# FraVirgu/Parallel-Geometric-Multigrid-for-Poisson-problem

Hardware: NVIDIA B200
Metric: V-cycle GDOF/s to 1e-8 residual (higher is better)
Workload: dtype f64

## Files before the change

### parallel-geometric-multigrid-for-poisson-problem_b200/csrc/kernels_fused.cu

```cuda
#include <cstdlib>
#include <cstring>

#define PMG_NEEDS_PEER_WAIT
#include "pmg_internal.h"

namespace pmg {

namespace {

constexpr int WARPS_PER_CTA = 4;

__host__ __device__ constexpr int halo_for(int stages) { return stages <= 4 ? 4 : 8; }

struct StripGeom {
    int n;
    int ny;
    int yoff;
    int row_lo;
    int row_hi;
    int pitch;
    int n_strips;
    int n_chunks;
    int chunk_rows;
    int halo;
// ... 125 lines not shown
        cen[p ^ 1] = in;
        return out;
    }
    template <bool WEIGHTED>
    __device__ __forceinline__ Row<C> step_wide(const int p, const Row<C> &in, const Row<C> &h2f, const JacobiCoef &c,
                                                bool keep0, bool keep_row)
    {
        static_assert(C == 4, "wide geometry: 4 columns per lane");
        Row<C> out, w, e;
        const Row<C> &prev = cen[p];
#pragma unroll
        for (int k = 0; k < C; ++k) {
            const double sum = dadd(part.v[k], in.v[k]);
            double val = WEIGHTED ? dadd(dmul(c.om1, prev.v[k]), dmul(c.w4, sum)) : dmul(0.25, sum);
            out.v[k] = ((k == 0) ? keep0 : keep_row) ? prev.v[k] : val;
        }
        neighbours<C>(in, w, e);
#pragma unroll
        for (int k = 0; k < C; ++k) part.v[k] = dadd(dadd(dadd(h2f.v[k], w.v[k]), e.v[k]), prev.v[k]);
        cen[p ^ 1] = in;
        return out;
    }
};

template <int C>
struct ResidualStage {
    Row<C> part;
    Row<C> cen[2];
    __device__ __forceinline__ void init()
    {
        cen[0] = zero_row<C>();
        cen[1] = zero_row<C>();
        part = zero_row<C>();
    }
    __device__ __forceinline__ Row<C> step(const int p, const Row<C> &in, const Row<C> &f_prev, double inv_h2)
    {
        Row<C> r, w, e;
#pragma unroll
        for (int k = 0; k < C; ++k)
            r.v[k] = dsub(f_prev.v[k], dmul(inv_h2, dsub(part.v[k], in.v[k])));
        neighbours<C>(in, w, e);
#pragma unroll
        for (int k = 0; k < C; ++k)
            part.v[k] = dsub(dsub(dfma_pow2(4.0, in.v[k], -w.v[k]), e.v[k]), cen[p].v[k]);
        cen[p ^ 1] = in;
        return r;
// ... 266 lines not shown
struct FeedSelect<C, PF, S, USE_X, true> {
    using type = SmemFeed<C, PF, S, USE_X>;
};

template <int C>
struct CoarseRow {
    double v[C / 2 + 1];
};

template <int C>
__device__ __forceinline__ CoarseRow<C> load_coarse(const double *__restrict__ p)
{
    CoarseRow<C> r;
    if (C == 4) {
        const double2 t = __ldg(reinterpret_cast<const double2 *>(p));
        r.v[0] = t.x;
        r.v[1] = t.y;
    } else {
        r.v[0] = __ldg(p);
    }
    return r;
}

template <int C, int PF, int MINB, bool SM, int S, bool ZEROX, bool RESID, bool WEIGHTED, bool PROLOGUE = false, bool PIN = false>
__global__ void __launch_bounds__(32 * WARPS_PER_CTA, MINB)
    k_down(const double *__restrict__ x, double *__restrict__ xo, const double *__restrict__ f,
           double *__restrict__ cf, StripGeom g, int pitch_c, int nc, JacobiCoef coef, double inv_h2,
           const int *__restrict__ done, HaloPeers hp, const double *__restrict__ e_in, int pitch_e, int lo)
{
    static_assert(!PIN || (ZEROX && SM), "prolong-in: the iterate is not read, shared-memory feed (row pairs)");
    using Feed = typename FeedSelect<C, PF, S, !ZEROX, SM>::type;
    pdl_wait();
    const bool pdl_early = gridDim.x <= 296u;
    if (pdl_early) pdl_trigger();
    if (done != nullptr && *done) return;
    constexpr int NP = C / 2;
    const int wid = __shfl_sync(0xffffffffu, (int)((blockIdx.x * (unsigned)blockDim.x + threadIdx.x) >> 5), 0);
    const int lane = threadIdx.x & 31;
    if (wid >= g.n_strips * g.n_chunks) return;
    int col, r0, r1;
    bool owner, cin[C];
    strip_setup<C>(g, wid, lane, col, r0, r1, owner, cin);

    const int lead = RESID ? 2 : 0;
    int j_start_ = min(r0, max(r0, 0) - lead) - S;
    if (PIN) j_start_ -= (j_start_ & 1);
    const int j_start = j_start_;
    const int j_end = max(r1 - 1, min(r1, g.ny) - 1 + (RESID ? 1 : 0)) + S;

    SweepStage<C> st[S];
    ResidualStage<C> rs;
#pragma unroll
    for (int k = 0; k < S; ++k) st[k].init();
    rs.init();
    double s_mid[NP], s_cor[NP], c_mid[NP], c_ew[NP];
#pragma unroll
    for (int q = 0; q < NP; ++q) s_mid[q] = s_cor[q] = c_mid[q] = c_ew[q] = 0.0;

    const int epoch = hp.epoch + (hp.epoch_base != nullptr ? *hp.epoch_base : 0);
    if ((hp.pub_up != nullptr || hp.pub_dn != nullptr) && blockIdx.x == 0 && threadIdx.x == 0) {
        __threadfence_system();
        if (hp.pub_up != nullptr) publish_epoch(hp.pub_up, epoch);
        if (hp.pub_dn != nullptr) publish_epoch(hp.pub_dn, epoch);
    }
    HaloPeers feed_peers = hp;
    if constexpr (!PROLOGUE) {
        if (hp.flag_up != nullptr || hp.flag_dn != nullptr) {
            int ok = 1;
            if (lane == 0) {
                if (hp.flag_up != nullptr) ok = wait_flag(hp.flag_up, epoch) ? ok : 0;
                if (hp.flag_dn != nullptr) ok = wait_flag(hp.flag_dn, epoch) ? ok : 0;
// ... 68 lines not shown
                double corr[C];
                if ((u & 1) == 0) {
                    en = eb;
                    en.v[NP] = __shfl_down_sync(0xffffffffu, eb.v[0], 1);
                    const int nr = min((jj >> 1) + 2, nc_last_row);
                    eb = load_coarse<C>(e_in + (ptrdiff_t)nr * pitch_e + cc);
#pragma unroll
                    for (int q = 0; q < NP; ++q) {
                        corr[2 * q] = ec.v[q];
                        corr[2 * q + 1] = dadd(ec.v[q], ec.v[q + 1]);
                    }
                } else {
#pragma unroll
                    for (int q = 0; q < NP; ++q) {
                        corr[2 * q] = dadd(ec.v[q], en.v[q]);
                        corr[2 * q + 1] = dadd(dadd(dadd(ec.v[q], ec.v[q + 1]), en.v[q]), en.v[q + 1]);
                    }
                    ec = en;
                }
#pragma unroll
                for (int k = 0; k < C; ++k)
                    if (rowp && cprol[k]) cur.v[k] = add_correction(cur.v[k], corr[k], u & 1, k & 1);
            }
#pragma unroll
            for (int k = 0; k < S; ++k) {
                const int out_row = jj - k - 1 + g.yoff;
                cur = st[k].template step<WEIGHTED>(u & 1, cur, feed.f_row(k), coef, out_row > 0 && out_row < g.n - 1, cin);
            }
            const int xrow = jj - S;
            if (owner && xrow >= r0 && xrow < r1) store_row<C>(xo + (ptrdiff_t)xrow * g.pitch + col, cur);
            if (RESID) {
                Row<C> r = rs.step(u & 1, cur, feed.f_row(S + 1), inv_h2);
                const int rrow = jj - S - 1;
                double left = __shfl_up_sync(0xffffffffu, r.v[C - 1], 1);
                if (rrow & 1) {
                    const int jc = (rrow - 1) >> 1;
                    const int ic = col >> 1;
                    double o[NP];
#pragma unroll
                    for (int q = 0; q < NP; ++q) {
                        double west = (q == 0) ? left : r.v[q == 0 ? 0 : 2 * q - 1];
                        double edge = dadd(dadd(c_ew[q], r.v[2 * q]), s_mid[q]);
                        double corner = dadd(dadd(s_cor[q], west), r.v[2 * q + 1]);
                        double val = dfma_pow2(0.0625, corner, dfma_pow2(0.125, edge, dmul(0.25, c_mid[q])));
                        o[q] = (ic + q >= 1 && ic + q < nc - 1) ? val : 0.0;
                        s_mid[q] = r.v[2 * q];
                        s_cor[q] = dadd(west, r.v[2 * q + 1]);
                    }
                    if (owner && jc + ycoarse >= 1 && jc + ycoarse < nc - 1 && 2 * jc >= r0 && 2 * jc < r1 &&
                        jc >= 0 && 2 * jc < g.ny) {
                        double *dst = cf + (ptrdiff_t)jc * pitch_c + ic;
                        if (NP == 2)
                            *reinterpret_cast<double2 *>(dst) = make_double2(o[0], o[NP - 1]);
                        else
                            *dst = o[0];
                    }
                } else {
#pragma unroll
                    for (int q = 0; q < NP; ++q) {
                        double west = (q == 0) ? left : r.v[q == 0 ? 0 : 2 * q - 1];
                        c_mid[q] = r.v[2 * q];
                        c_ew[q] = dadd(r.v[2 * q + 1], west);
                    }
                }
            }
            feed.end();
        }
    }
    if (!pdl_early) pdl_trigger();
    cp_async_wait<0>();
}

template <int C, int PF, int MINB, bool SM, int S, bool PROLONG, bool NORM, bool WEIGHTED>
__global__ void __launch_bounds__(32 * WARPS_PER_CTA, MINB)
    k_up(const double *__restrict__ xb, double *__restrict__ xo, const double *__restrict__ f,
         const double *__restrict__ e, StripGeom g, int pitch_c, int lo, JacobiCoef coef, double inv_h2,
         double *__restrict__ partials, const int *__restrict__ done)
{
    using Feed = typename FeedSelect<C, PF, S, true, SM>::type;
    pdl_wait();
    const bool pdl_early = gridDim.x <= 296u;
    if (pdl_early) pdl_trigger();
    if (done != nullptr && *done) return;
    static_assert(Feed::UNROLL % 2 == 0, "rows are processed in (even, odd) pairs");
    constexpr int NP = C / 2;
    const int wid = __shfl_sync(0xffffffffu, (int)((blockIdx.x * (unsigned)blockDim.x + threadIdx.x) >> 5), 0);
    const int lane = threadIdx.x & 31;
    if (wid >= g.n_strips * g.n_chunks) return;
    int col, r0, r1;
    bool owner, cin[C];
    strip_setup<C>(g, wid, lane, col, r0, r1, owner, cin);

    int j_start = r0 - S - (NORM ? 1 : 0);
    j_start -= (j_start & 1);
    const int j_end = r1 - 1 + S + (NORM ? 1 : 0);

    SweepStage<C> st[S];
    ResidualStage<C> rs;
#pragma unroll
    for (int k = 0; k < S; ++k) st[k].init();
    rs.init();
    double acc = 0.0;

    bool cprol[C];
#pragma unroll
    for (int k = 0; k < C; ++k) cprol[k] = (col + k >= lo) && (col + k <= g.n - 2);

    Feed feed;
    feed.init(xb, f, g.pitch, col, j_start, g.ny + PADY - 1, lane, threadIdx.x >> 5, HaloPeers{}, g.ny);

    const int cc = col >> 1;
    const int nc_last_row = ((g.ny - 1) >> 1) + PADY;
    CoarseRow<C> ec, en, eb;
#pragma unroll
    for (int q = 0; q <= NP; ++q) ec.v[q] = en.v[q] = eb.v[q] = 0.0;
    if (PROLONG) {
        const int jc0 = j_start >> 1;
        ec = load_coarse<C>(e + (ptrdiff_t)jc0 * pitch_c + cc);
        ec.v[NP] = __shfl_down_sync(0xffffffffu, ec.v[0], 1);
        eb = load_coarse<C>(e + (ptrdiff_t)(jc0 + 1) * pitch_c + cc);
    }

    for (int j = j_start; j <= j_end; j += Feed::UNROLL) {
#pragma unroll
        for (int u = 0; u < Feed::UNROLL; ++u) {
            const int jj = j + u;
            Row<C> cur = feed.begin(u, jj);
            if (PROLONG) {
                const bool rowp = (jj + g.yoff >= lo) && (jj + g.yoff <= g.n - 2);
                double corr[C];
                if ((u & 1) == 0) {
                    en = eb;
                    en.v[NP] = __shfl_down_sync(0xffffffffu, eb.v[0], 1);
                    int nr = min((jj >> 1) + 2, nc_last_row);
                    eb = load_coarse<C>(e + (ptrdiff_t)nr * pitch_c + cc);
#pragma unroll
                    for (int q = 0; q < NP; ++q) {
                        corr[2 * q] = ec.v[q];
                        corr[2 * q + 1] = dadd(ec.v[q], ec.v[q + 1]);
                    }
                } else {
#pragma unroll
                    for (int q = 0; q < NP; ++q) {
                        corr[2 * q] = dadd(ec.v[q], en.v[q]);
                        corr[2 * q + 1] = dadd(dadd(dadd(ec.v[q], ec.v[q + 1]), en.v[q]), en.v[q + 1]);
                    }
                    ec = en;
                }
#pragma unroll
                for (int k = 0; k < C; ++k)
                    if (rowp && cprol[k]) cur.v[k] = add_correction(cur.v[k], corr[k], u & 1, k & 1);
            }
#pragma unroll
            for (int k = 0; k < S; ++k) {
                const int out_row = jj - k - 1 + g.yoff;
                cur = st[k].template step<WEIGHTED>(u & 1, cur, feed.f_row(k), coef, out_row > 0 && out_row < g.n - 1, cin);
            }
            const int xrow = jj - S;
            if (owner && xrow >= r0 && xrow < r1) store_row<C>(xo + (ptrdiff_t)xrow * g.pitch + col, cur);
            if (NORM) {
                Row<C> r = rs.step(u & 1, cur, feed.f_row(S + 1), inv_h2);
                const int rrow = jj - S - 1;
                if (owner && rrow >= r0 && rrow < r1 && rrow >= 0 && rrow < g.ny && rrow + g.yoff > 0 &&
                    rrow + g.yoff < g.n - 1) {
#pragma unroll
                    for (int k = 0; k < C; ++k)
                        if (cin[k]) acc = dadd(acc, dmul(r.v[k], r.v[k]));
                }
            }
            feed.end();
        }
    }
    if (!pdl_early) pdl_trigger();
    cp_async_wait<0>();
    if (NORM) {
#pragma unroll
        for (int o = 16; o > 0; o >>= 1) acc = dadd(acc, __shfl_xor_sync(0xffffffffu, acc, o));
        if (lane == 0) partials[wid] = acc;
    }
}

template <int C, int PF, int MINB, int S2, int S1, bool WEIGHTED, bool GEN_F = false>
__global__ void __launch_bounds__(32 * WARPS_PER_CTA, MINB)
    k_cross(const double *__restrict__ xb, double *__restrict__ xo, double *__restrict__ xk, const double *__restrict__ f,
// ... 289 lines not shown
#endif

inline int current_device()
{
#ifdef PMG_HOST_EMULATION
    return 0;
#else
    int d = 0;
    cudaGetDevice(&d);
    return d & 63;
#endif
}
#define PMG_SMEM_ONCE(k, sm)                         \
    do {                                             \
        static unsigned long long mask_ = 0;         \
        const int d_ = current_device();             \
        if (!((mask_ >> d_) & 1ull)) {               \
            set_smem(k, sm);                         \
            mask_ |= 1ull << d_;                     \
        }                                            \
    } while (0)

template <int C, int PF, int MINB, bool SM, int S, bool WEIGHTED>
void down_launch_w(const FusedLevel &lv, double *cf, int pitch_c, bool x_is_zero, bool resid, const StripGeom &g,
                   int nc, const JacobiCoef &c, double inv, dim3 grid, dim3 block, const int *done, cudaStream_t st)
{
    constexpr bool CAN_PROLOGUE = SM && S == 2;
    const bool prologue = CAN_PROLOGUE && g_halo_prologue && (lv.hp.flag_up != nullptr || lv.hp.flag_dn != nullptr);
    if (resid && x_is_zero && prologue) {
        auto k = k_down<C, PF, MINB, SM, S, true, true, WEIGHTED, CAN_PROLOGUE>;
        int sm = WARPS_PER_CTA * FeedSelect<C, PF, S, false, SM>::type::SMEM_PER_WARP;
        PMG_SMEM_ONCE(k, sm);
        PMG_LAUNCH(k, grid, block, sm, st, lv.x, lv.xb, lv.f, cf, g, pitch_c, nc, c, inv, done, lv.hp, (const double *)nullptr, 0, 0);
    } else if (resid && prologue) {
        auto k = k_down<C, PF, MINB, SM, S, false, true, WEIGHTED, CAN_PROLOGUE>;
        int sm = WARPS_PER_CTA * FeedSelect<C, PF, S, true, SM>::type::SMEM_PER_WARP;
        PMG_SMEM_ONCE(k, sm);
        PMG_LAUNCH(k, grid, block, sm, st, lv.x, lv.xb, lv.f, cf, g, pitch_c, nc, c, inv, done, lv.hp, (const double *)nullptr, 0, 0);
    } else if (resid && x_is_zero) {
        auto k = k_down<C, PF, MINB, SM, S, true, true, WEIGHTED>;
        int sm = WARPS_PER_CTA * FeedSelect<C, PF, S, false, SM>::type::SMEM_PER_WARP;
        PMG_SMEM_ONCE(k, sm);
        PMG_LAUNCH(k, grid, block, sm, st, lv.x, lv.xb, lv.f, cf, g, pitch_c, nc, c, inv, done, lv.hp, (const double *)nullptr, 0, 0);
    } else if (resid) {
        auto k = k_down<C, PF, MINB, SM, S, false, true, WEIGHTED>;
        int sm = WARPS_PER_CTA * FeedSelect<C, PF, S, true, SM>::type::SMEM_PER_WARP;
        PMG_SMEM_ONCE(k, sm);
        PMG_LAUNCH(k, grid, block, sm, st, lv.x, lv.xb, lv.f, cf, g, pitch_c, nc, c, inv, done, lv.hp, (const double *)nullptr, 0, 0);
    } else {
        auto k = k_down<C, PF, MINB, SM, S, false, false, WEIGHTED>;
        int sm = WARPS_PER_CTA * FeedSelect<C, PF, S, true, SM>::type::SMEM_PER_WARP;
        PMG_SMEM_ONCE(k, sm);
        PMG_LAUNCH(k, grid, block, sm, st, lv.x, lv.xb, lv.f, (double *)nullptr, g, 0, nc, c, inv, done, lv.hp, (const double *)nullptr, 0, 0);
    }
}

template <int C, int PF, int MINB, bool SM, int S>
void down_launch(const FusedLevel &lv, double *cf, int pitch_c, double omega, bool x_is_zero, bool resid,
                 const int *done, cudaStream_t st)
{
    StripGeom g = make_geom(lv, S + (resid ? 2 : 0), VariantDesc{C, PF, MINB, SM}, lv.ext_lo, lv.ext_hi);
    JacobiCoef c = jacobi_coef(lv.h, omega);
    double inv = 1.0 / (lv.h * lv.h);
    int nc = (lv.n - 1) / 2 + 1;
    dim3 grid(grid_for(g)), block(32 * WARPS_PER_CTA);
    if (c.weighted) {
        down_launch_w<C, PF, MINB, SM, S, true>(lv, cf, pitch_c, x_is_zero, resid, g, nc, c, inv, grid, block, done, st);
    } else {
        down_launch_w<C, PF, MINB, SM, S, false>(lv, cf, pitch_c, x_is_zero, resid, g, nc, c, inv, grid, block, done, st);
    }
    count_launch();
}

template <bool WEIGHTED>
void down_prolong_launch_w(const FusedLevel &lv, const double *e_in, int pitch_e, int lo, double *cf, int pitch_c,
                           const JacobiCoef &c, const int *done, cudaStream_t st)
{
    constexpr int C = 2, PF = 3, MINB = 5, S = 2;
    StripGeom g = make_geom(lv, S + 2, VariantDesc{C, PF, MINB, 1}, lv.ext_lo, lv.ext_hi);
    const double inv = 1.0 / (lv.h * lv.h);
    const int nc = (lv.n - 1) / 2 + 1;
    auto k = k_down<C, PF, MINB, true, S, true, true, WEIGHTED, false, true>;
    int sm = WARPS_PER_CTA * SmemFeed<C, PF, S, false>::SMEM_PER_WARP;
    PMG_SMEM_ONCE(k, sm);
    PMG_LAUNCH(k, dim3(grid_for(g)), dim3(32 * WARPS_PER_CTA), sm, st, lv.x, lv.xb, lv.f, cf, g, pitch_c, nc, c, inv, done,
               HaloPeers{}, e_in, pitch_e, lo);
}

template <int C, int PF, int MINB, bool SM, int S, bool PROLONG, bool NORM, bool WEIGHTED>
void up_launch_k(const FusedLevel &lv, const double *e, int pitch_c, const StripGeom &g, int lo,
                 const JacobiCoef &c, double inv, double *d_partials, const int *done, cudaStream_t st)
{
    auto k = k_up<C, PF, MINB, SM, S, PROLONG, NORM, WEIGHTED>;
    int sm = WARPS_PER_CTA * FeedSelect<C, PF, S, true, SM>::type::SMEM_PER_WARP;
    PMG_SMEM_ONCE(k, sm);
    PMG_LAUNCH(k, dim3(grid_for(g)), dim3(32 * WARPS_PER_CTA), sm, st, lv.xb, lv.x, lv.f, e, g, pitch_c, lo, c, inv, d_partials, done);
}

template <int C, int PF, int MINB, bool SM, int S, bool PROLONG, bool NORM>
void up_launch_one(const FusedLevel &lv, const double *e, int pitch_c, const StripGeom &g, int lo,
                   const JacobiCoef &c, double inv, double *d_partials, const int *done, cudaStream_t st)
{
    if (c.weighted)
        up_launch_k<C, PF, MINB, SM, S, PROLONG, NORM, true>(lv, e, pitch_c, g, lo, c, inv, d_partials, done, st);
    else
        up_launch_k<C, PF, MINB, SM, S, PROLONG, NORM, false>(lv, e, pitch_c, g, lo, c, inv, d_partials, done, st);
}

template <int C, int PF, int MINB, bool SM, int S>
void up_launch(const FusedLevel &lv, const double *e, int pitch_c, double omega, int lo, bool norm,
               double *d_partials, int *n_partials, const int *done, cudaStream_t st)
{
    StripGeom g = make_geom(lv, S + (norm ? 2 : 1), VariantDesc{C, PF, MINB, SM}, lv.ext_lo, lv.ext_hi);
    JacobiCoef c = jacobi_coef(lv.h, omega);
    double inv = 1.0 / (lv.h * lv.h);
    if (e != nullptr) {
        if (norm)
            up_launch_one<C, PF, MINB, SM, S, true, true>(lv, e, pitch_c, g, lo, c, inv, d_partials, done, st);
        else
            up_launch_one<C, PF, MINB, SM, S, true, false>(lv, e, pitch_c, g, lo, c, inv, d_partials, done, st);
    } else {
        if (norm)
            up_launch_one<C, PF, MINB, SM, S, false, true>(lv, e, pitch_c, g, lo, c, inv, d_partials, done, st);
        else
            up_launch_one<C, PF, MINB, SM, S, false, false>(lv, e, pitch_c, g, lo, c, inv, d_partials, done, st);
    }
    count_launch();
    if (n_partials) *n_partials = norm ? g.n_strips * g.n_chunks : 0;
}

template <int C, int PF, int MINB, bool WEIGHTED, bool GEN_F = false>
void cross_launch_w(const FusedLevel &lv_in, double *xb_out, const double *e, int pitch_c, double *cf, int lo, double *d_partials,
                    int *n_partials, const JacobiCoef &c, const int *done, cudaStream_t st)
{
    VariantDesc v{C, PF, MINB, 1};
    StripGeom g = make_geom(lv_in, 6, v, 0, 0, C == 2 ? 6 : 8);
    double inv = 1.0 / (lv_in.h * lv_in.h);
    int nc = (lv_in.n - 1) / 2 + 1;
    auto k = k_cross<C, PF, MINB, 2, 2, WEIGHTED, GEN_F>;
    int sm = WARPS_PER_CTA * SmemFeed<C, PF, 4, true, GEN_F, C == 4>::SMEM_PER_WARP;
    PMG_SMEM_ONCE(k, sm);
    PMG_LAUNCH(k, dim3(grid_for(g)), dim3(32 * WARPS_PER_CTA), sm, st, lv_in.xb, xb_out, lv_in.x, lv_in.f, e, cf, g, pitch_c, lo, nc, c,
               inv, d_partials, done, lv_in.hp, lv_in.rhs_fx, lv_in.rhs_sy);
    if (n_partials) *n_partials = g.n_strips * g.n_chunks;
}

}

bool fused_supported(int nu) { return nu >= 1 && nu <= 4; }
int fused_take_bad_nu()
{
// ... 57 lines not shown
        PMG_CROSS(6);
    else
        PMG_CROSS(3);
#undef PMG_CROSS
    count_launch();
}

int fused_num_variants() { return NUM_VARIANTS; }
void fused_set_variant(int v)
{
    int d = v & 0xff, u = (v >> 8) & 0xff;
    if (!(v & 0x10000)) u = d;
    g_variant_down = g_variant_down_zero = (d >= 0 && d < NUM_VARIANTS) ? d : 0;
    g_variant_up = g_variant_up_norm = (u >= 0 && u < NUM_VARIANTS) ? u : 0;
    if (v < 0) {
        g_variant_down = 0;
        g_variant_down_zero = 3;
        g_variant_up = 1;
        g_variant_up_norm = 3;
    }
}
int fused_get_variant() { return g_variant_down | (g_variant_up << 8); }
void fused_set_min_chunk_rows(int r) { g_min_chunk_rows = (r >= 2) ? (r + (r & 1)) : 2; }
void fused_set_deep_prefetch_below(int n) { g_deep_prefetch_below = n; }
void fused_set_halo_prologue(int on) { g_halo_prologue = on ? 1 : 0; }
void fused_set_wait_timeout_ns(unsigned long long ns)
{
#ifndef PMG_HOST_EMULATION
    cudaMemcpyToSymbol(g_wait_timeout_ns, &ns, sizeof(ns));
#else
    (void)ns;
#endif
}
int fused_halo_prologue() { return g_halo_prologue; }

int fused_max_partials(int n)
{
    int best = 0;
    FusedLevel lv{};
    lv.n = n;
    lv.pitch = level_pitch(n);
    for (int v = 0; v < NUM_VARIANTS; ++v) {
        StripGeom g = make_geom(lv, 8, VARIANTS[v], 8, 8);
        int c = g.n_strips * g.n_chunks;
        g = make_geom(lv, 4, VARIANTS[v], 8, 8);
        if (g.n_strips * g.n_chunks > c) c = g.n_strips * g.n_chunks;
        if (c > best) best = c;
    }
    return best + 64;
}

#define PMG_DISPATCH_S2(VAR, FN, ...)                                       \
    switch (VAR) {                                                          \
        case 1: FN<2, 3, 5, true, 2>(__VA_ARGS__); break;                   \
        case 2: FN<2, 4, 4, false, 2>(__VA_ARGS__); break;                  \
        case 3: FN<2, 3, 6, true, 2>(__VA_ARGS__); break;                   \
        case 4: FN<2, 7, 4, true, 2>(__VA_ARGS__); break;                   \
        default: FN<2, 3, 4, true, 2>(__VA_ARGS__); break;                  \
    }

void launch_fused_down(const FusedLevel &lv, double *coarse_f, int pitch_c, int nu1, double omega,
                       bool x_is_zero, cudaStream_t st, const int *done)
{
    bool resid = coarse_f != nullptr;
    if (!fused_supported(nu1)) {
        g_fused_bad_nu = nu1;
        return;
    }
    switch (nu1) {
        case 1: down_launch<2, 3, 4, true, 1>(lv, coarse_f, pitch_c, omega, x_is_zero, resid, done, st); break;
        case 2: PMG_DISPATCH_S2(lv.n <= deep_prefetch_below() ? 4 : ((x_is_zero && resid) ? g_variant_down_zero : g_variant_down), down_launch, lv, coarse_f, pitch_c, omega, x_is_zero, resid, done, st); break;
        case 3: down_launch<2, 3, 4, true, 3>(lv, coarse_f, pitch_c, omega, x_is_zero, resid, done, st); break;
        case 4: down_launch<2, 2, 4, true, 4>(lv, coarse_f, pitch_c, omega, x_is_zero, resid, done, st); break;
        default: break;
    }
}

bool fused_down_prolong_supported(int nu1) { return nu1 == 2; }
void launch_fused_down_prolong(const FusedLevel &lv, const double *e_in, int pitch_e, double *coarse_f, int pitch_c, double omega,
                               int prolong_mode, cudaStream_t st, const int *done)
{
    const int lo = prolong_mode == PMG_PROLONG_FULL ? 1 : 2;
    JacobiCoef c = jacobi_coef(lv.h, omega);
    if (c.weighted)
        down_prolong_launch_w<true>(lv, e_in, pitch_e, lo, coarse_f, pitch_c, c, done, st);
    else
        down_prolong_launch_w<false>(lv, e_in, pitch_e, lo, coarse_f, pitch_c, c, done, st);
    count_launch();
}

void launch_fused_up(const FusedLevel &lv, const double *coarse_x, int pitch_c, int nu2, double omega,
                     int prolong_mode, double *d_partials, int *n_partials, cudaStream_t st, const int *done)
{
    bool norm = d_partials != nullptr;
    int lo = prolong_mode == PMG_PROLONG_FULL ? 1 : 2;
    if (!fused_supported(nu2)) {
        g_fused_bad_nu = nu2;
        if (n_partials) *n_partials = 0;
        return;
    }
    switch (nu2) {
        case 1: up_launch<2, 3, 4, true, 1>(lv, coarse_x, pitch_c, omega, lo, norm, d_partials, n_partials, done, st); break;
        case 2: PMG_DISPATCH_S2(lv.n <= deep_prefetch_below() ? 4 : (norm ? g_variant_up_norm : g_variant_up), up_launch, lv, coarse_x, pitch_c, omega, lo, norm, d_partials, n_partials, done, st); break;
        case 3: up_launch<2, 3, 4, true, 3>(lv, coarse_x, pitch_c, omega, lo, norm, d_partials, n_partials, done, st); break;
        case 4: up_launch<2, 2, 4, true, 4>(lv, coarse_x, pitch_c, omega, lo, norm, d_partials, n_partials, done, st); break;
        default: break;
    }
}

}
```

### parallel-geometric-multigrid-for-poisson-problem_b200/csrc/pmg_internal.h

```cpp
#pragma once
#if defined(PMG_HOST_EMULATION) && defined(__CUDACC__)
#error "PMG_HOST_EMULATION is for the g++-compiled kernel tests under tests/cpp only; libpmg.so is never built with it"
#endif
#ifdef PMG_HOST_EMULATION
#include "host_emulation.h"
#else
#include <cuda_runtime.h>
#endif

#include <cstddef>
#include <cstdint>

#include "pmg.h"

namespace pmg {

constexpr int PADX = 16;
constexpr int PADY = 8;

inline int level_pitch(int n) { return ((PADX + n + 144) + 15) / 16 * 16; }
inline size_t level_elems(int n) { return (size_t)level_pitch(n) * (size_t)(n + 2 * PADY); }
inline size_t level_origin(int n) { return (size_t)PADY * level_pitch(n) + PADX; }

__device__ __forceinline__ double dadd(double a, double b) { return __dadd_rn(a, b); }
// ... 182 lines not shown
                return false;
        }
    }
}
#endif

struct FusedLevel {
    double *x;
    double *xb;
    const double *f;
    int n, pitch;
    double h;
    int ny, yoff, ext_lo, ext_hi;
    int span_lo, span_hi;
    HaloPeers hp;
    const double *rhs_fx, *rhs_sy;
};
bool fused_supported(int nu);
bool fused_down_prolong_supported(int nu1);
void launch_fused_down_prolong(const FusedLevel &lv, const double *e_in, int pitch_e, double *coarse_f, int pitch_c, double omega,
                               int prolong_mode, cudaStream_t st, const int *done = nullptr);
int fused_take_bad_nu();
void launch_fused_down(const FusedLevel &lv, double *coarse_f, int pitch_c, int nu1, double omega,
                       bool x_is_zero, cudaStream_t st, const int *done = nullptr);
void launch_fused_up(const FusedLevel &lv, const double *coarse_x, int pitch_c, int nu2, double omega,
                     int prolong_mode, double *d_partials, int *n_partials, cudaStream_t st,
                     const int *done = nullptr);
int fused_max_partials(int n);
bool fused_cross_supported(int nu1, int nu2);
double fused_cross_utilisation(int n, int rows);
void launch_fused_cross(const FusedLevel &lv, double *xb_out, const double *coarse_x, double *coarse_f, int pitch_c, double omega,
                        int prolong_mode, double *d_partials, int *n_partials, cudaStream_t st, const int *done = nullptr);
void fused_set_cross_minb(int m);
int fused_num_variants();
void fused_set_variant(int v);
int fused_get_variant();
void fused_set_min_chunk_rows(int r);
constexpr int PMG_DEEP_PREFETCH_DEFAULT = 0;
void fused_set_deep_prefetch_below(int n);
constexpr int PMG_HALO_PROLOGUE_DEFAULT = 1;
void fused_set_halo_prologue(int on);
int fused_halo_prologue();
void fused_set_wait_timeout_ns(unsigned long long ns);
void basic_set_wait_timeout_ns(unsigned long long ns);

bool comm_ready();
int comm_rank();
int comm_size();
pmg_status comm_halo_exchange(double *p, int ny, int pitch, int depth, cudaStream_t st);
pmg_status comm_gather_rows(const double *slab, double *full, int pitch, const int *y0s, const int *y1s,
// ... 26 lines not shown
```

### parallel-geometric-multigrid-for-poisson-problem_b200/csrc/solver.cu

```cuda
#include <cmath>
#include <cstdio>
#include <cstdlib>
#include <cstring>
#include <mutex>
#include <new>
#include <string>
#include <vector>

#include "pmg_internal.h"

#include <execinfo.h>
#include <fcntl.h>
#include <signal.h>
#include <unistd.h>

namespace pmg {

static int g_debug_fd = -1;
static void pmg_signal_handler(int sig)
{
    void *frames[64];
    int n = backtrace(frames, 64);
    const char msg[] = "\n[libpmg] fatal signal, native backtrace:\n";
    (void)!write(g_debug_fd, msg, sizeof(msg) - 1);
// ... 295 lines not shown
    }
    launch_prolong_add(K.x, L.x, K.n, L.n, K.pitch, L.pitch, c.prolong_mode, s->stream);
    return smooth_operator(s, l, c.nu2, false);
}

static pmg_status cycle_fused(pmg_solver *s, int l, bool w_form, bool x_is_zero, bool want_norm, int *n_partials,
                              const int *done = nullptr, const Level *prolong_in = nullptr)
{
    const pmg_config &c = s->cfg;
    Level &L = s->lv[l];
    if (L.n <= c.n_coarse || l + 1 == (int)s->lv.size())
        return smooth_operator(s, l, c.coarse_sweeps, x_is_zero, done);
    if (l > 0 && L.n == s->cluster_top &&
        launch_coarse_cluster(L.x, L.f, L.n, L.pitch, L.pitch, c.n_coarse, L.h, c.omega, c.nu1, c.nu2, c.coarse_sweeps,
                              c.prolong_mode, x_is_zero, w_form ? c.gamma : 1, s->stream, done))
        return PMG_OK;
    if (l > 0 && L.n <= VSMALL_TOP && s->small_vcycle && (int)s->lv.size() - l <= 8 &&
        s->lv.back().n * s->lv.back().n <= SMALL_MAX_POINTS) {
        launch_vcycle_small(L.x, L.f, L.n, L.pitch, L.pitch, c.n_coarse, L.h, c.omega, c.nu1, c.nu2, c.coarse_sweeps,
                            c.prolong_mode, x_is_zero, w_form ? c.gamma : 1, s->stream, done);
        return PMG_OK;
    }
    Level &K = s->lv[l + 1];
    if (prolong_in != nullptr)
        launch_fused_down_prolong(fused_view(L), prolong_in->x, prolong_in->pitch, K.f, K.pitch, c.omega, c.prolong_mode,
                                  s->stream, done);
    else
        launch_fused_down(fused_view(L), K.f, K.pitch, c.nu1, c.omega, x_is_zero, s->stream, done);
    int reps = w_form ? c.gamma : 1;
    for (int k = 0; k < reps; ++k) {
        pmg_status rc = cycle_fused(s, l + 1, w_form, k == 0, false, nullptr, done);
        if (rc != PMG_OK) return rc;
    }
    launch_fused_up(fused_view(L), K.x, K.pitch, c.nu2, c.omega, c.prolong_mode,
                    want_norm ? s->d_partials : nullptr, n_partials, s->stream, done);
    return PMG_OK;
}

static bool fused_graph_ok(const pmg_solver *s);

static pmg_status coarse_solve_redundant(pmg_solver *s, bool w_form, int reps)
{
    auto direct = [&]() -> pmg_status {
        for (int k = 0; k < reps; ++k) {
            pmg_status rc = cycle_fused(s, s->agg_level, w_form, k == 0, false, nullptr, nullptr);
            if (rc != PMG_OK) return rc;
        }
        return PMG_OK;
    };
    if (!s->coarse_graph_on || !fused_graph_ok(s) || s->capturing_mid) return direct();
    cudaGraphExec_t &ge = s->coarse_graph[w_form ? 1 : 0];
    int &gk = s->coarse_graph_kernels[w_form ? 1 : 0];
    if (ge == nullptr) {
        const unsigned long long before = launches_so_far();
        PMG_CUDA(cudaStreamBeginCapture(s->stream, cudaStreamCaptureModeThreadLocal));
        pmg_status rc = direct();
        cudaGraph_t g = nullptr;
        cudaError_t e = cudaStreamEndCapture(s->stream, &g);
// ... 1718 lines not shown
    for (auto &m : g_trace) cudaEventDestroy(m.ev);
    g_trace.clear();
}

void pmg_small_vcycle_set_version(int v) { vcycle_small_set_version(v); }
int pmg_small_vcycle_version(void) { return vcycle_small_version(); }

void pmg_set_pdl(int on) { pdl_set_enabled(on); }

void pmg_set_cross_cycle(int on) { g_cross_override = on < 0 ? -1 : (on >= 2 ? 2 : (on ? 1 : 0)); }
int pmg_cross_cycle_active(const pmg_solver *s)
{
    if (!s) return 0;
    return s->dist ? (cross_ok_dist(s, false) ? 1 : 0) : (cross_ok(s, false) ? 1 : 0);
}
void pmg_fused_set_cross_minb(int m) { fused_set_cross_minb(m); }

void pmg_set_cluster_top(int n) { g_cluster_override = (n == 257 || n == 129 || n == 0) ? n : -1; }
int pmg_cluster_top(const pmg_solver *s) { return s ? s->cluster_top : 0; }

int pmg_fused_num_variants(void) { return fused_num_variants(); }
void pmg_fused_set_variant(int v) { fused_set_variant(v); }
void pmg_fused_set_min_chunk_rows(int r) { fused_set_min_chunk_rows(r); }
void pmg_fused_set_deep_prefetch_below(int n) { fused_set_deep_prefetch_below(n); }
void pmg_fused_set_halo_prologue(int on) { fused_set_halo_prologue(on); }

pmg_status pmg_bench_small(int n0, int gamma, int reps, int version, double *us_avg)
{
    const bool cluster = coarse_cluster_top(n0);
    if (!us_avg || reps < 1 || gamma < 1 || n0 < 3 || (n0 > VSMALL_TOP && !cluster) || ((n0 - 1) & (n0 - 2)) != 0)
        return fail(PMG_ERR_INVALID, "bad argument");
    if (pmg_device_count() <= 0) return fail(PMG_ERR_NO_DEVICE, "no CUDA device visible; this library has no CPU fallback");
    const int pitch = level_pitch(n0);
    double *x = nullptr, *f = nullptr;
    pmg_status rc = alloc_zero(&x, level_elems(n0));
    if (rc == PMG_OK) rc = alloc_zero(&f, level_elems(n0));
    if (rc != PMG_OK) {
        cudaFree(x);
        return rc;
    }
    launch_fill2d(f + level_origin(n0) + pitch + 1, pitch, n0 - 2, n0 - 2, 1.0, nullptr);
    const int before = vcycle_small_version();
    vcycle_small_set_version(version);
    cudaStream_t st = nullptr;
    cudaEvent_t e0 = nullptr, e1 = nullptr;
    cudaStreamCreate(&st);
// ... 65 lines not shown
}

pmg_status pmg_bench_pass(pmg_solver *s, int which, int level, int reps, double *ms_avg)
{
    if (!s || !ms_avg || reps < 1 || level < 0 || level + 1 >= (int)s->lv.size() || !s->fused)
        return fail(PMG_ERR_INVALID, "bad argument (needs the fused engine and a non-coarsest level)");
    PMG_CUDA(cudaSetDevice(s->device));
    Level &L = s->lv[level];
    Level &K = s->lv[level + 1];
    const pmg_config &c = s->cfg;
    int np = 0;
    if (which == 4) {
        if (level != 0 || s->dist || !fused_cross_supported(c.nu1, c.nu2))
            return fail(PMG_ERR_UNSUPPORTED, "cross-cycle pass: level 0, one GPU, nu1 = nu2 = 2");
        pmg_status rcx = ensure_xc(s);
        if (rcx != PMG_OK) return rcx;
    }
    auto one = [&]() {
        if (which == 4) {
            FusedLevel v = fused_view(L);
            v.x = nullptr;
            use_rhs_tables(s, v);
            launch_fused_cross(v, s->xc, K.x, K.f, K.pitch, c.omega, c.prolong_mode, s->d_partials, &np, s->stream);
        } else if (which == 0 || which == 3)
            launch_fused_down(fused_view(L), K.f, K.pitch, c.nu1, c.omega, which == 3, s->stream);
        else
            launch_fused_up(fused_view(L), K.x, K.pitch, c.nu2, c.omega, c.prolong_mode,
                            which == 1 ? s->d_partials : nullptr, &np, s->stream);
    };
    one();
    PMG_CUDA(cudaEventRecord(s->ev0, s->stream));
    for (int i = 0; i < reps; ++i) one();
    PMG_CUDA(cudaEventRecord(s->ev1, s->stream));
    PMG_CUDA(cudaEventSynchronize(s->ev1));
    PMG_CUDA(cudaGetLastError());
    float ms = 0.f;
    PMG_CUDA(cudaEventElapsedTime(&ms, s->ev0, s->ev1));
    *ms_avg = ms / reps;
    return PMG_OK;
}

static pmg_status require_device();

typedef struct {
    double *x, *xb;
    const double *f;
    int n, pitch;
    double h;
    int ny, yoff, ext_lo, ext_hi, span_lo, span_hi;
    const double *x_up, *x_dn, *f_up, *f_dn;
    double *f_keep, *x_keep;
    int *flag_up, *flag_dn, *pub_up, *pub_dn;
    int epoch;
    int *err;
} pmg_test_slab;

void pmg_test_layout(int n, int *pitch, int *padx, int *pady)
{
    if (pitch) *pitch = level_pitch(n);
    if (padx) *padx = PADX;
// ... 382 lines not shown
```

Measured before the change: 2.640.

## Rebuild pre-smoothed iterate in up-pass instead of storing it on large levels

```diff
diff --git a/parallel-geometric-multigrid-for-poisson-problem_b200/csrc/kernels_fused.cu b/parallel-geometric-multigrid-for-poisson-problem_b200/csrc/kernels_fused.cu
--- a/parallel-geometric-multigrid-for-poisson-problem_b200/csrc/kernels_fused.cu
+++ b/parallel-geometric-multigrid-for-poisson-problem_b200/csrc/kernels_fused.cu
@@ -171,6 +171,23 @@
         return out;
     }
 };
+
+template <bool WEIGHTED>
+__device__ __forceinline__ double sweep_from_zero(double f, const JacobiCoef &c)
+{
+    const double sum = dadd(dmul(c.h2, f), 0.0);
+    return WEIGHTED ? dadd(dmul(c.om1, 0.0), dmul(c.w4, sum)) : dmul(0.25, sum);
+}
+
+template <int C, bool WEIGHTED>
+__device__ __forceinline__ Row<C> sweep_row_from_zero(const Row<C> &f_row, const JacobiCoef &c, bool row_interior,
+                                                      const bool (&col_interior)[C])
+{
+    Row<C> out;
+#pragma unroll
+    for (int k = 0; k < C; ++k) out.v[k] = (row_interior && col_interior[k]) ? sweep_from_zero<WEIGHTED>(f_row.v[k], c) : 0.0;
+    return out;
+}
 
 template <int C>
 struct ResidualStage {
@@ -483,13 +500,17 @@
     return r;
 }
 
-template <int C, int PF, int MINB, bool SM, int S, bool ZEROX, bool RESID, bool WEIGHTED, bool PROLOGUE = false, bool PIN = false>
+template <int C, int PF, int MINB, bool SM, int S, bool ZEROX, bool RESID, bool WEIGHTED, bool PROLOGUE = false, bool PIN = false,
+          bool NO_XB = false>
 __global__ void __launch_bounds__(32 * WARPS_PER_CTA, MINB)
     k_down(const double *__restrict__ x, double *__restrict__ xo, const double *__restrict__ f,
            double *__restrict__ cf, StripGeom g, int pitch_c, int nc, JacobiCoef coef, double inv_h2,
            const int *__restrict__ done, HaloPeers hp, const double *__restrict__ e_in, int pitch_e, int lo)
 {
     static_assert(!PIN || (ZEROX && SM), "prolong-in: the iterate is not read, shared-memory feed (row pairs)");
+    static_assert(!NO_XB || (ZEROX && RESID && !PIN), "xb is rebuilt by Pass B only on a first visit");
+    constexpr bool PW = ZEROX && !PIN;
+    constexpr int SD = PW ? S - 1 : S;
     using Feed = typename FeedSelect<C, PF, S, !ZEROX, SM>::type;
     pdl_wait();
     const bool pdl_early = gridDim.x <= 296u;
@@ -504,10 +525,10 @@
     strip_setup<C>(g, wid, lane, col, r0, r1, owner, cin);
 
     const int lead = RESID ? 2 : 0;
-    int j_start_ = min(r0, max(r0, 0) - lead) - S;
+    int j_start_ = min(r0, max(r0, 0) - lead) - SD;
     if (PIN) j_start_ -= (j_start_ & 1);
     const int j_start = j_start_;
-    const int j_end = max(r1 - 1, min(r1, g.ny) - 1 + (RESID ? 1 : 0)) + S;
+    const int j_end = max(r1 - 1, min(r1, g.ny) - 1 + (RESID ? 1 : 0)) + SD;
 
     SweepStage<C> st[S];
     ResidualStage<C> rs;
@@ -622,16 +643,18 @@
                 for (int k = 0; k < C; ++k)
                     if (rowp && cprol[k]) cur.v[k] = add_correction(cur.v[k], corr[k], u & 1, k & 1);
             }
-#pragma unroll
-            for (int k = 0; k < S; ++k) {
+            if (PW)
+                cur = sweep_row_from_zero<C, WEIGHTED>(feed.f_row(0), coef, jj + g.yoff > 0 && jj + g.yoff < g.n - 1, cin);
+#pragma unroll
+            for (int k = 0; k < SD; ++k) {
                 const int out_row = jj - k - 1 + g.yoff;
                 cur = st[k].template step<WEIGHTED>(u & 1, cur, feed.f_row(k), coef, out_row > 0 && out_row < g.n - 1, cin);
             }
-            const int xrow = jj - S;
-            if (owner && xrow >= r0 && xrow < r1) store_row<C>(xo + (ptrdiff_t)xrow * g.pitch + col, cur);
+            const int xrow = jj - SD;
+            if (!NO_XB && owner && xrow >= r0 && xrow < r1) store_row<C>(xo + (ptrdiff_t)xrow * g.pitch + col, cur);
             if (RESID) {
-                Row<C> r = rs.step(u & 1, cur, feed.f_row(S + 1), inv_h2);
-                const int rrow = jj - S - 1;
+                Row<C> r = rs.step(u & 1, cur, feed.f_row(SD + 1), inv_h2);
+                const int rrow = jj - SD - 1;
                 double left = __shfl_up_sync(0xffffffffu, r.v[C - 1], 1);
                 if (rrow & 1) {
                     const int jc = (rrow - 1) >> 1;
@@ -671,13 +694,14 @@
     cp_async_wait<0>();
 }
 
-template <int C, int PF, int MINB, bool SM, int S, bool PROLONG, bool NORM, bool WEIGHTED>
+template <int C, int PF, int MINB, bool SM, int S, bool PROLONG, bool NORM, bool WEIGHTED, int REBUILD = 0>
 __global__ void __launch_bounds__(32 * WARPS_PER_CTA, MINB)
     k_up(const double *__restrict__ xb, double *__restrict__ xo, const double *__restrict__ f,
          const double *__restrict__ e, StripGeom g, int pitch_c, int lo, JacobiCoef coef, double inv_h2,
          double *__restrict__ partials, const int *__restrict__ done)
 {
-    using Feed = typename FeedSelect<C, PF, S, true, SM>::type;
+    constexpr int D1 = REBUILD > 0 ? REBUILD - 1 : 0;
+    using Feed = typename FeedSelect<C, PF, S + D1, REBUILD == 0, SM>::type;
     pdl_wait();
     const bool pdl_early = gridDim.x <= 296u;
     if (pdl_early) pdl_trigger();
@@ -691,10 +715,15 @@
     bool owner, cin[C];
     strip_setup<C>(g, wid, lane, col, r0, r1, owner, cin);
 
-    int j_start = r0 - S - (NORM ? 1 : 0);
+    int j_start = r0 - S - (NORM ? 1 : 0) - 2 * D1;
+    if (REBUILD > 0) j_start = max(j_start, -PADY - D1);
     j_start -= (j_start & 1);
+    if (REBUILD > 0 && j_start + D1 < -PADY) j_start += 2;
     const int j_end = r1 - 1 + S + (NORM ? 1 : 0);
 
+    SweepStage<C> pre[D1 > 0 ? D1 : 1];
+#pragma unroll
+    for (int k = 0; k < D1; ++k) pre[k].init();
     SweepStage<C> st[S];
     ResidualStage<C> rs;
 #pragma unroll
@@ -707,7 +736,7 @@
     for (int k = 0; k < C; ++k) cprol[k] = (col + k >= lo) && (col + k <= g.n - 2);
 
     Feed feed;
-    feed.init(xb, f, g.pitch, col, j_start, g.ny + PADY - 1, lane, threadIdx.x >> 5, HaloPeers{}, g.ny);
+    feed.init(xb, f, g.pitch, col, j_start + D1, g.ny + PADY - 1, lane, threadIdx.x >> 5, HaloPeers{}, g.ny);
 
     const int cc = col >> 1;
     const int nc_last_row = ((g.ny - 1) >> 1) + PADY;
@@ -725,7 +754,15 @@
 #pragma unroll
         for (int u = 0; u < Feed::UNROLL; ++u) {
             const int jj = j + u;
-            Row<C> cur = feed.begin(u, jj);
+            Row<C> cur = feed.begin(u, jj + D1);
+            if (REBUILD > 0) {
+                cur = sweep_row_from_zero<C, WEIGHTED>(feed.f_row(0), coef, jj + D1 + g.yoff > 0 && jj + D1 + g.yoff < g.n - 1, cin);
+#pragma unroll
+                for (int k = 0; k < D1; ++k) {
+                    const int out_row = jj + D1 - k - 1 + g.yoff;
+                    cur = pre[k].template step<WEIGHTED>(u & 1, cur, feed.f_row(k), coef, out_row > 0 && out_row < g.n - 1, cin);
+                }
+            }
             if (PROLONG) {
                 const bool rowp = (jj + g.yoff >= lo) && (jj + g.yoff <= g.n - 2);
                 double corr[C];
@@ -754,12 +791,12 @@
 #pragma unroll
             for (int k = 0; k < S; ++k) {
                 const int out_row = jj - k - 1 + g.yoff;
-                cur = st[k].template step<WEIGHTED>(u & 1, cur, feed.f_row(k), coef, out_row > 0 && out_row < g.n - 1, cin);
+                cur = st[k].template step<WEIGHTED>(u & 1, cur, feed.f_row(D1 + k), coef, out_row > 0 && out_row < g.n - 1, cin);
             }
             const int xrow = jj - S;
             if (owner && xrow >= r0 && xrow < r1) store_row<C>(xo + (ptrdiff_t)xrow * g.pitch + col, cur);
             if (NORM) {
-                Row<C> r = rs.step(u & 1, cur, feed.f_row(S + 1), inv_h2);
+                Row<C> r = rs.step(u & 1, cur, feed.f_row(D1 + S + 1), inv_h2);
                 const int rrow = jj - S - 1;
                 if (owner && rrow >= r0 && rrow < r1 && rrow >= 0 && rrow < g.ny && rrow + g.yoff > 0 &&
                     rrow + g.yoff < g.n - 1) {
@@ -1095,7 +1132,7 @@
     } while (0)
 
 template <int C, int PF, int MINB, bool SM, int S, bool WEIGHTED>
-void down_launch_w(const FusedLevel &lv, double *cf, int pitch_c, bool x_is_zero, bool resid, const StripGeom &g,
+void down_launch_w(const FusedLevel &lv, double *cf, int pitch_c, bool x_is_zero, bool resid, bool store_xb, const StripGeom &g,
                    int nc, const JacobiCoef &c, double inv, dim3 grid, dim3 block, const int *done, cudaStream_t st)
 {
     constexpr bool CAN_PROLOGUE = SM && S == 2;
@@ -1108,6 +1145,11 @@
     } else if (resid && prologue) {
         auto k = k_down<C, PF, MINB, SM, S, false, true, WEIGHTED, CAN_PROLOGUE>;
         int sm = WARPS_PER_CTA * FeedSelect<C, PF, S, true, SM>::type::SMEM_PER_WARP;
+        PMG_SMEM_ONCE(k, sm);
+        PMG_LAUNCH(k, grid, block, sm, st, lv.x, lv.xb, lv.f, cf, g, pitch_c, nc, c, inv, done, lv.hp, (const double *)nullptr, 0, 0);
+    } else if (resid && x_is_zero && !store_xb) {
+        auto k = k_down<C, PF, MINB, SM, S, true, true, WEIGHTED, false, false, true>;
+        int sm = WARPS_PER_CTA * FeedSelect<C, PF, S, false, SM>::type::SMEM_PER_WARP;
         PMG_SMEM_ONCE(k, sm);
         PMG_LAUNCH(k, grid, block, sm, st, lv.x, lv.xb, lv.f, cf, g, pitch_c, nc, c, inv, done, lv.hp, (const double *)nullptr, 0, 0);
     } else if (resid && x_is_zero) {
@@ -1129,7 +1171,7 @@
 }
 
 template <int C, int PF, int MINB, bool SM, int S>
-void down_launch(const FusedLevel &lv, double *cf, int pitch_c, double omega, bool x_is_zero, bool resid,
+void down_launch(const FusedLevel &lv, double *cf, int pitch_c, double omega, bool x_is_zero, bool resid, bool store_xb,
                  const int *done, cudaStream_t st)
 {
     StripGeom g = make_geom(lv, S + (resid ? 2 : 0), VariantDesc{C, PF, MINB, SM}, lv.ext_lo, lv.ext_hi);
@@ -1138,9 +1180,9 @@
     int nc = (lv.n - 1) / 2 + 1;
     dim3 grid(grid_for(g)), block(32 * WARPS_PER_CTA);
     if (c.weighted) {
-        down_launch_w<C, PF, MINB, SM, S, true>(lv, cf, pitch_c, x_is_zero, resid, g, nc, c, inv, grid, block, done, st);
+        down_launch_w<C, PF, MINB, SM, S, true>(lv, cf, pitch_c, x_is_zero, resid, store_xb, g, nc, c, inv, grid, block, done, st);
     } else {
-        down_launch_w<C, PF, MINB, SM, S, false>(lv, cf, pitch_c, x_is_zero, resid, g, nc, c, inv, grid, block, done, st);
+        down_launch_w<C, PF, MINB, SM, S, false>(lv, cf, pitch_c, x_is_zero, resid, store_xb, g, nc, c, inv, grid, block, done, st);
     }
     count_launch();
 }
@@ -1160,12 +1202,12 @@
                HaloPeers{}, e_in, pitch_e, lo);
 }
 
-template <int C, int PF, int MINB, bool SM, int S, bool PROLONG, bool NORM, bool WEIGHTED>
+template <int C, int PF, int MINB, bool SM, int S, bool PROLONG, bool NORM, bool WEIGHTED, int REBUILD = 0>
 void up_launch_k(const FusedLevel &lv, const double *e, int pitch_c, const StripGeom &g, int lo,
                  const JacobiCoef &c, double inv, double *d_partials, const int *done, cudaStream_t st)
 {
-    auto k = k_up<C, PF, MINB, SM, S, PROLONG, NORM, WEIGHTED>;
-    int sm = WARPS_PER_CTA * FeedSelect<C, PF, S, true, SM>::type::SMEM_PER_WARP;
+    auto k = k_up<C, PF, MINB, SM, S, PROLONG, NORM, WEIGHTED, REBUILD>;
+    int sm = WARPS_PER_CTA * FeedSelect<C, PF, S + (REBUILD > 0 ? REBUILD - 1 : 0), REBUILD == 0, SM>::type::SMEM_PER_WARP;
     PMG_SMEM_ONCE(k, sm);
     PMG_LAUNCH(k, dim3(grid_for(g)), dim3(32 * WARPS_PER_CTA), sm, st, lv.xb, lv.x, lv.f, e, g, pitch_c, lo, c, inv, d_partials, done);
 }
@@ -1200,6 +1242,32 @@
     }
     count_launch();
     if (n_partials) *n_partials = norm ? g.n_strips * g.n_chunks : 0;
+}
+
+template <int C, int PF, int MINB, bool SM, int S, int NU1>
+void up_rebuild_launch(const FusedLevel &lv, const double *e, int pitch_c, double omega, int lo, const int *done, cudaStream_t st)
+{
+    StripGeom g = make_geom(lv, (NU1 - 1) + S + 1, VariantDesc{C, PF, MINB, SM}, lv.ext_lo, lv.ext_hi);
+    JacobiCoef c = jacobi_coef(lv.h, omega);
+    double inv = 1.0 / (lv.h * lv.h);
+    if (c.weighted)
+        up_launch_k<C, PF, MINB, SM, S, true, false, true, NU1>(lv, e, pitch_c, g, lo, c, inv, nullptr, done, st);
+    else
+        up_launch_k<C, PF, MINB, SM, S, true, false, false, NU1>(lv, e, pitch_c, g, lo, c, inv, nullptr, done, st);
+    count_launch();
+}
+
+template <int C, int PF, int MINB, bool SM, int S>
+void up_rebuild_dispatch(const FusedLevel &lv, const double *e, int pitch_c, double omega, int lo, int nu1, const int *done,
+                         cudaStream_t st)
+{
+    switch (nu1) {
+        case 1: up_rebuild_launch<C, PF, MINB, SM, S, 1>(lv, e, pitch_c, omega, lo, done, st); break;
+        case 2: up_rebuild_launch<C, PF, MINB, SM, S, 2>(lv, e, pitch_c, omega, lo, done, st); break;
+        case 3: up_rebuild_launch<C, PF, MINB, SM, S, 3>(lv, e, pitch_c, omega, lo, done, st); break;
+        case 4: up_rebuild_launch<C, PF, MINB, SM, S, 4>(lv, e, pitch_c, omega, lo, done, st); break;
+        default: break;
+    }
 }
 
 template <int C, int PF, int MINB, bool WEIGHTED, bool GEN_F = false>
@@ -1303,6 +1371,33 @@
 }
 int fused_get_variant() { return g_variant_down | (g_variant_up << 8); }
 void fused_set_min_chunk_rows(int r) { g_min_chunk_rows = (r >= 2) ? (r + (r & 1)) : 2; }
+
+int g_rebuild_xb = -2;
+void fused_set_rebuild_xb(int mode) { g_rebuild_xb = (mode == 0 || mode == 1) ? mode : -1; }
+static size_t l2_bytes()
+{
+#ifdef PMG_HOST_EMULATION
+    return (size_t)126 << 20;
+#else
+    int dev = 0, v = 0;
+    cudaGetDevice(&dev);
+    static int cached[64] = {};
+    int &c = cached[dev & 63];
+    if (c == 0) c = (cudaDeviceGetAttribute(&v, cudaDevAttrL2CacheSize, dev) == cudaSuccess && v > 0) ? v : -1;
+    return c > 0 ? (size_t)c : 0;
+#endif
+}
+bool fused_rebuild_xb(const FusedLevel &lv, int nu1)
+{
+    if (g_rebuild_xb == -2) {
+        const char *e = getenv("PMG_REBUILD_XB");
+        g_rebuild_xb = (e && (e[0] == '0' || e[0] == '1')) ? e[0] - '0' : -1;
+    }
+    if (lv.ny != 0 || !fused_supported(nu1) || g_rebuild_xb == 0) return false;
+    if (g_rebuild_xb == 1) return true;
+    const size_t l2 = l2_bytes();
+    return l2 > 0 && 3 * level_elems(lv.n) * sizeof(double) > l2;
+}
 void fused_set_deep_prefetch_below(int n) { g_deep_prefetch_below = n; }
 void fused_set_halo_prologue(int on) { g_halo_prologue = on ? 1 : 0; }
 void fused_set_wait_timeout_ns(unsigned long long ns)
@@ -1341,18 +1436,18 @@
     }
 
 void launch_fused_down(const FusedLevel &lv, double *coarse_f, int pitch_c, int nu1, double omega,
-                       bool x_is_zero, cudaStream_t st, const int *done)
+                       bool x_is_zero, cudaStream_t st, const int *done, bool store_xb)
 {
     bool resid = coarse_f != nullptr;
-    if (!fused_supported(nu1)) {
-        g_fused_bad_nu = nu1;
+    if (!fused_supported(nu1) || (!store_xb && !(x_is_zero && resid && lv.ny == 0))) {
+        g_fused_bad_nu = fused_supported(nu1) ? -1 : nu1;
         return;
     }
     switch (nu1) {
-        case 1: down_launch<2, 3, 4, true, 1>(lv, coarse_f, pitch_c, omega, x_is_zero, resid, done, st); break;
-        case 2: PMG_DISPATCH_S2(lv.n <= deep_prefetch_below() ? 4 : ((x_is_zero && resid) ? g_variant_down_zero : g_variant_down), down_launch, lv, coarse_f, pitch_c, omega, x_is_zero, resid, done, st); break;
-        case 3: down_launch<2, 3, 4, true, 3>(lv, coarse_f, pitch_c, omega, x_is_zero, resid, done, st); break;
-        case 4: down_launch<2, 2, 4, true, 4>(lv, coarse_f, pitch_c, omega, x_is_zero, resid, done, st); break;
+        case 1: down_launch<2, 3, 4, true, 1>(lv, coarse_f, pitch_c, omega, x_is_zero, resid, store_xb, done, st); break;
+        case 2: PMG_DISPATCH_S2(lv.n <= deep_prefetch_below() ? 4 : ((x_is_zero && resid) ? g_variant_down_zero : g_variant_down), down_launch, lv, coarse_f, pitch_c, omega, x_is_zero, resid, store_xb, done, st); break;
+        case 3: down_launch<2, 3, 4, true, 3>(lv, coarse_f, pitch_c, omega, x_is_zero, resid, store_xb, done, st); break;
+        case 4: down_launch<2, 2, 4, true, 4>(lv, coarse_f, pitch_c, omega, x_is_zero, resid, store_xb, done, st); break;
         default: break;
     }
 }
@@ -1371,7 +1466,7 @@
 }
 
 void launch_fused_up(const FusedLevel &lv, const double *coarse_x, int pitch_c, int nu2, double omega,
-                     int prolong_mode, double *d_partials, int *n_partials, cudaStream_t st, const int *done)
+                     int prolong_mode, double *d_partials, int *n_partials, cudaStream_t st, const int *done, int rebuild_nu1)
 {
     bool norm = d_partials != nullptr;
     int lo = prolong_mode == PMG_PROLONG_FULL ? 1 : 2;
@@ -1380,6 +1475,21 @@
         if (n_partials) *n_partials = 0;
         return;
     }
+    if (rebuild_nu1 != 0) {
+        if (n_partials) *n_partials = 0;
+        if (!fused_supported(rebuild_nu1) || norm || coarse_x == nullptr || lv.ny != 0) {
+            g_fused_bad_nu = fused_supported(rebuild_nu1) ? -1 : rebuild_nu1;
+            return;
+        }
+        switch (nu2) {
+            case 1: up_rebuild_dispatch<2, 3, 4, true, 1>(lv, coarse_x, pitch_c, omega, lo, rebuild_nu1, done, st); break;
+            case 2: up_rebuild_dispatch<2, 3, 5, true, 2>(lv, coarse_x, pitch_c, omega, lo, rebuild_nu1, done, st); break;
+            case 3: up_rebuild_dispatch<2, 3, 4, true, 3>(lv, coarse_x, pitch_c, omega, lo, rebuild_nu1, done, st); break;
+            case 4: up_rebuild_dispatch<2, 2, 4, true, 4>(lv, coarse_x, pitch_c, omega, lo, rebuild_nu1, done, st); break;
+            default: break;
+        }
+        return;
+    }
     switch (nu2) {
         case 1: up_launch<2, 3, 4, true, 1>(lv, coarse_x, pitch_c, omega, lo, norm, d_partials, n_partials, done, st); break;
         case 2: PMG_DISPATCH_S2(lv.n <= deep_prefetch_below() ? 4 : (norm ? g_variant_up_norm : g_variant_up), up_launch, lv, coarse_x, pitch_c, omega, lo, norm, d_partials, n_partials, done, st); break;
diff --git a/parallel-geometric-multigrid-for-poisson-problem_b200/csrc/pmg_internal.h b/parallel-geometric-multigrid-for-poisson-problem_b200/csrc/pmg_internal.h
--- a/parallel-geometric-multigrid-for-poisson-problem_b200/csrc/pmg_internal.h
+++ b/parallel-geometric-multigrid-for-poisson-problem_b200/csrc/pmg_internal.h
@@ -228,10 +228,12 @@
                                int prolong_mode, cudaStream_t st, const int *done = nullptr);
 int fused_take_bad_nu();
 void launch_fused_down(const FusedLevel &lv, double *coarse_f, int pitch_c, int nu1, double omega,
-                       bool x_is_zero, cudaStream_t st, const int *done = nullptr);
+                       bool x_is_zero, cudaStream_t st, const int *done = nullptr, bool store_xb = true);
 void launch_fused_up(const FusedLevel &lv, const double *coarse_x, int pitch_c, int nu2, double omega,
                      int prolong_mode, double *d_partials, int *n_partials, cudaStream_t st,
-                     const int *done = nullptr);
+                     const int *done = nullptr, int rebuild_nu1 = 0);
+bool fused_rebuild_xb(const FusedLevel &lv, int nu1);
+void fused_set_rebuild_xb(int mode);
 int fused_max_partials(int n);
 bool fused_cross_supported(int nu1, int nu2);
 double fused_cross_utilisation(int n, int rows);
diff --git a/parallel-geometric-multigrid-for-poisson-problem_b200/csrc/solver.cu b/parallel-geometric-multigrid-for-poisson-problem_b200/csrc/solver.cu
--- a/parallel-geometric-multigrid-for-poisson-problem_b200/csrc/solver.cu
+++ b/parallel-geometric-multigrid-for-poisson-problem_b200/csrc/solver.cu
@@ -341,18 +341,19 @@
         return PMG_OK;
     }
     Level &K = s->lv[l + 1];
+    const bool rebuild = prolong_in == nullptr && x_is_zero && !want_norm && fused_rebuild_xb(fused_view(L), c.nu1);
     if (prolong_in != nullptr)
         launch_fused_down_prolong(fused_view(L), prolong_in->x, prolong_in->pitch, K.f, K.pitch, c.omega, c.prolong_mode,
                                   s->stream, done);
     else
-        launch_fused_down(fused_view(L), K.f, K.pitch, c.nu1, c.omega, x_is_zero, s->stream, done);
+        launch_fused_down(fused_view(L), K.f, K.pitch, c.nu1, c.omega, x_is_zero, s->stream, done, !rebuild);
     int reps = w_form ? c.gamma : 1;
     for (int k = 0; k < reps; ++k) {
         pmg_status rc = cycle_fused(s, l + 1, w_form, k == 0, false, nullptr, done);
         if (rc != PMG_OK) return rc;
     }
     launch_fused_up(fused_view(L), K.x, K.pitch, c.nu2, c.omega, c.prolong_mode,
-                    want_norm ? s->d_partials : nullptr, n_partials, s->stream, done);
+                    want_norm ? s->d_partials : nullptr, n_partials, s->stream, done, rebuild ? c.nu1 : 0);
     return PMG_OK;
 }
 
@@ -2117,6 +2118,7 @@
 int pmg_fused_num_variants(void) { return fused_num_variants(); }
 void pmg_fused_set_variant(int v) { fused_set_variant(v); }
 void pmg_fused_set_min_chunk_rows(int r) { fused_set_min_chunk_rows(r); }
+void pmg_fused_set_rebuild_xb(int mode) { fused_set_rebuild_xb(mode); }
 void pmg_fused_set_deep_prefetch_below(int n) { fused_set_deep_prefetch_below(n); }
 void pmg_fused_set_halo_prologue(int on) { fused_set_halo_prologue(on); }
 
@@ -2228,11 +2230,11 @@
             v.x = nullptr;
             use_rhs_tables(s, v);
             launch_fused_cross(v, s->xc, K.x, K.f, K.pitch, c.omega, c.prolong_mode, s->d_partials, &np, s->stream);
-        } else if (which == 0 || which == 3)
-            launch_fused_down(fused_view(L), K.f, K.pitch, c.nu1, c.omega, which == 3, s->stream);
+        } else if (which == 0 || which == 3 || which == 5)
+            launch_fused_down(fused_view(L), K.f, K.pitch, c.nu1, c.omega, which != 0, s->stream, nullptr, which != 5);
         else
             launch_fused_up(fused_view(L), K.x, K.pitch, c.nu2, c.omega, c.prolong_mode,
-                            which == 1 ? s->d_partials : nullptr, &np, s->stream);
+                            which == 1 ? s->d_partials : nullptr, &np, s->stream, nullptr, which == 6 ? c.nu1 : 0);
     };
     one();
     PMG_CUDA(cudaEventRecord(s->ev0, s->stream));
@@ -2242,6 +2244,7 @@
     PMG_CUDA(cudaGetLastError());
     float ms = 0.f;
     PMG_CUDA(cudaEventElapsedTime(&ms, s->ev0, s->ev1));
+    if (fused_take_bad_nu()) return fail(PMG_ERR_UNSUPPORTED, "this pass form needs a whole level (one GPU)");
     *ms_avg = ms / reps;
     return PMG_OK;
 }
```

New measurement: 2.732, median of 6. 1.03x the previous value.
